# NVIDIA-Genomics-Research/GenomeWorks

Hardware: AMD Instinct MI355X
Metric: cudapoa consensus GCUPS, 1024-window short-read batch (static band 256, 32 reads <= 1024 bp) (higher is better)
Workload: dtype int16; 1 GPU; BASELINE configs[2]: cudapoa single-batch consensus, 1024 windows x 32 reads, backbone 960 bp, <=48 sub/24 ins/24 del, BatchConfig(1024,32,256,static_band), scores 8/-6/-8; windows_per_gpu=1024, cells_per_gpu=10990578176, parallelism=index-split x1

## Files before the change

### genomeworks_amd/csrc/gwhip_poa.hip

```cpp
#include <hip/hip_runtime.h>

#include <cstdio>
#include <cstdlib>
#include <cstring>
#include <string>

#include "poa_device.h"
#include "poa_full_device.h"
#include "poa_graph_device.h"
#include "poa_tb_device.h"

namespace gwhip
{

#ifndef GWHIP_POA_PART
thread_local std::string g_last_error;

static int fail(hipError_t e, const char* what)
{
    g_last_error = std::string(what) + ": " + hipGetErrorString(e);
    return (int)e;
}
static int fail_msg(int code, const std::string& msg)
{
// ... 182 lines not shown
    uint64_t phase_acc[kPhCount] = {0, 0, 0, 0, 0, 0};
    PhaseClock pc{(DBG && a.phase_cycles) ? phase_acc : nullptr, 0};
    wave_sync();
    pc.start();

    for (int32_t s = 1; s < (int32_t)wd.num_seqs; s++)
    {
        const int32_t seq_len = seq_lens[s];
        const int32_t adv     = ((s == 1 ? len0 : seq_lens[s - 1]) + 3) & ~3;
        sequence += adv;
        base_weights += adv;

        if (node_count >= c.max_nodes_per_graph)
        {
            if (lane == 0) { consensus[0] = kKernelError; consensus[1] = kNodeCountExceeded; }
            break;
        }
        pc.tick(kPhOther);
        build_rowinfo<IdT, RowT>(g, node_count, rowinfo, lane, LDS_TABLES ? reinterpret_cast<uint64_t*>(lds_code_tile) : nullptr);
        constexpr bool LDS_READ = LDS_TABLES && BM != GWHIP_FULL_BAND;
        const uint8_t* lds_read = lds_read_buf;
        if constexpr (LDS_READ)
        {
            const int32_t stage_bytes = min(kReadLds, ((max(seq_len, kMaxAdaptiveBand) + 8) + 3) & ~3);
            for (int32_t i = lane * 4; i < stage_bytes; i += kWave * 4)
                *reinterpret_cast<uint32_t*>(lds_read_buf + i) = *reinterpret_cast<const uint32_t*>(sequence + i);
        }
        wave_sync();
        pc.tick(kPhRowInfo);

        int32_t alen = 0;
        constexpr bool kTbPacked = TB && LDS_TABLES && std::is_same<ScoreT, int16_t>::value && std::is_same<TraceT, int16_t>::value;
        bool tb_handled = false;
        if constexpr (kTbPacked)
        {
            constexpr bool kAd = BM == GWHIP_ADAPTIVE_BAND_TRACEBACK;
            const bool adaptive_now = kAd && c.alignment_band_width < kMaxAdaptiveBand;
            auto packed = [&](auto ad_tag, int32_t rerun) -> int32_t {
                return nw_banded_tb_packed<IdT, decltype(ad_tag)::value>(g, rowinfo, node_count, lds_read, seq_len, reinterpret_cast<int16_t*>(scores),
                                                                         a.L.scores_elems, reinterpret_cast<int16_t*>(traceback), a.L.trace_elems,
                                                                         banded_buffer_size, alignment_graph, alignment_read, c.alignment_band_width,
                                                                         c.max_banded_pred_distance, c.gap_score, c.mismatch_score, c.match_score, rerun,
                                                                         cells, smem, kRingBytes, reinterpret_cast<const uint64_t*>(lds_code_tile),
                                                                         debug_flags, tb_handled);
            };
            if (adaptive_now)
                alen = packed(std::integral_constant<bool, kAd>{}, 0);
            else
                alen = packed(std::false_type{}, 0);
        }
        if (tb_handled && !(alen == kShiftLeft || alen == kShiftRight)) {}
        else if (BM == GWHIP_ADAPTIVE_BAND_TRACEBACK && c.alignment_band_width < kMaxAdaptiveBand)
// ... 3 lines not shown
                                                               traceback, a.L.trace_elems, banded_buffer_size, alignment_graph,
                                                               alignment_read, c.alignment_band_width, c.max_banded_pred_distance,
                                                               c.gap_score, c.mismatch_score, c.match_score, alen, cells);
            else
            alen = nw_banded_tb<ScoreT, IdT, RowT, TraceT, true>(g, rowinfo, node_count, sequence, seq_len, scores, a.L.scores_elems,
                                                           traceback, a.L.trace_elems, banded_buffer_size, alignment_graph,
                                                           alignment_read, c.alignment_band_width, c.max_banded_pred_distance,
                                                           c.gap_score, c.mismatch_score, c.match_score, 0, cells);
            if (alen == kShiftLeft || alen == kShiftRight)
                alen = nw_banded_tb<ScoreT, IdT, RowT, TraceT, true>(g, rowinfo, node_count, sequence, seq_len, scores, a.L.scores_elems,
                                                               traceback, a.L.trace_elems, banded_buffer_size, alignment_graph,
                                                               alignment_read, c.alignment_band_width, c.max_banded_pred_distance,
                                                               c.gap_score, c.mismatch_score, c.match_score, alen, cells);
        }
        else if (TB)
        {
            alen = nw_banded_tb<ScoreT, IdT, RowT, TraceT, false>(g, rowinfo, node_count, sequence, seq_len, scores, a.L.scores_elems,
                                                            traceback, a.L.trace_elems, banded_buffer_size, alignment_graph,
                                                            alignment_read, c.alignment_band_width, c.max_banded_pred_distance,
                                                            c.gap_score, c.mismatch_score, c.match_score, 0, cells);
        }
        else if (BM == GWHIP_ADAPTIVE_BAND && c.alignment_band_width < kMaxAdaptiveBand)
        {
            alen = nw_banded<ScoreT, IdT, RowT, true, LDS_READ, PV>(g, rowinfo, node_count, sequence, lds_read, seq_len, scores, ring, ring_bytes,
                                                banded_buffer_size, alignment_graph, alignment_read, c.alignment_band_width,
                                                c.gap_score, c.mismatch_score, c.match_score, 0, cells, pc, debug_flags, codes, lds_code_tile, lds_read_window, lds_bs_ring,
                                                mw_args, mw_shared);
            if (alen == kShiftLeft || alen == kShiftRight)
                alen = nw_banded<ScoreT, IdT, RowT, true, LDS_READ, PV>(g, rowinfo, node_count, sequence, lds_read, seq_len, scores, ring, ring_bytes,
                                                    banded_buffer_size, alignment_graph, alignment_read,
                                                    c.alignment_band_width, c.gap_score, c.mismatch_score, c.match_score,
                                                    alen, cells, pc, debug_flags, codes, lds_code_tile, lds_read_window, lds_bs_ring,
                                                    mw_args, mw_shared);
        }
        else if (BM == GWHIP_STATIC_BAND || BM == GWHIP_ADAPTIVE_BAND)
        {
            alen = nw_banded<ScoreT, IdT, RowT, false, LDS_READ, PV>(g, rowinfo, node_count, sequence, lds_read, seq_len, scores, ring, ring_bytes,
                                                 banded_buffer_size, alignment_graph, alignment_read, c.alignment_band_width,
                                                 c.gap_score, c.mismatch_score, c.match_score, 0, cells, pc, debug_flags, codes, lds_code_tile, lds_read_window, lds_bs_ring);
        }
        else
        {
            bool full_handled = false;
            if constexpr (kFullPacked)
                alen = nw_full_packed<IdT>(g, rowinfo, node_count, sequence, seq_len, reinterpret_cast<int16_t*>(scores), wd.scores_width, full_moves,
                                           smem, kRingBytes, reinterpret_cast<const uint64_t*>(lds_code_tile), alignment_graph, alignment_read,
                                           c.gap_score, c.mismatch_score, c.match_score, cells, debug_flags, full_handled, pc);
            if (!full_handled)
                alen = nw_full<ScoreT, IdT, RowT>(g, rowinfo, node_count, sequence, seq_len, scores, wd.scores_width, ring, kRingBytes,
                                            alignment_graph, alignment_read, c.gap_score, c.mismatch_score, c.match_score, cells);
        }
        alen = (int32_t)(IdT)alen;

        uint8_t err = 0;
        if (alen == kNwLoopFailed) err = kLoopCountExceeded;
        else if (alen == kNwAdaptiveStorageFailed) err = kExceededAdaptiveBandedMatrixSize;
        else if (TB && alen == kNwTracebackBufferFailed) err = kExceededMaximumPredecessorDistance;
        else if (alen == kNwPipelineFailed || alen == kNwScoreWrapped) err = kGenericError;
        if (err)
        {
// ... 6 lines not shown
        int32_t par_rc           = -1;
        if constexpr (!LDS_TABLES && !TB && BM != GWHIP_FULL_BAND)
        {
            int32_t new_count   = 0;
            int32_t* scratch    = reinterpret_cast<int32_t*>(scores);
            const int32_t lpad  = (seq_len + 63) & ~63;
            par_rc = add_alignment_parallel<IdT, MSA, int32_t>(new_count, g, node_count, alen, alignment_graph, alignment_read,
                                                               sequence, base_weights, seq_len, MSA ? g.seq_begin + s : nullptr,
                                                               (uint16_t)s, (uint32_t)c.max_sequences_per_poa,
                                                               c.max_nodes_per_graph, scratch, scratch + lpad,
                                                               reinterpret_cast<uint32_t*>(scratch + 2 * lpad), lane,
                                                               debug_flags, pc.acc ? &pc.acc[kPhOther] : nullptr);
            if (par_rc == 0)
            {
                if (lane == 0) seq_lens[0] = new_count;
                status_and_count = new_count;
            }
            else if (par_rc > 0)
            {
                if (lane == 0) { consensus[0] = kKernelError; consensus[1] = (uint8_t)par_rc; }
                status_and_count = -1;
            }
        }
        if constexpr (LDS_TABLES)
        {
            int32_t new_count = 0;
            par_rc = add_alignment_parallel<IdT, MSA>(new_count, g, node_count, alen, alignment_graph, alignment_read,
                                                      sequence, base_weights, seq_len, MSA ? g.seq_begin + s : nullptr,
                                                      (uint16_t)s, (uint32_t)c.max_sequences_per_poa,
                                                      c.max_nodes_per_graph, reinterpret_cast<int16_t*>(smem),
                                                      reinterpret_cast<int16_t*>(smem) + 2048,
                                                      reinterpret_cast<uint32_t*>(lds_rowinfo_region), lane, debug_flags,
                                                      pc.acc ? &pc.acc[kPhOther] : nullptr);
            if (par_rc == 0)
            {
                if (lane == 0) seq_lens[0] = new_count;
                status_and_count = new_count;
            }
            else if (par_rc > 0)
            {
                if (lane == 0) { consensus[0] = kKernelError; consensus[1] = (uint8_t)par_rc; }
                status_and_count = -1;
            }
        }
        if (lane == 0 && par_rc < 0)
        {
            int32_t new_count = 0;
            uint8_t e = add_alignment_to_graph<IdT, MSA>(new_count, g, node_count, alen, alignment_graph, sequence,
                                                         alignment_read, base_weights, MSA ? g.seq_begin + s : nullptr,
                                                         (uint16_t)s, (uint32_t)c.max_sequences_per_poa,
                                                         (uint32_t)c.max_nodes_per_graph);
            if (e != 0)
            {
                consensus[0]     = kKernelError;
                consensus[1]     = e;
                status_and_count = -1;
            }
            else
            {
                seq_lens[0]      = new_count;
                status_and_count = new_count;
            }
        }
        pc.tick(kPhAddAlignment);
        status_and_count = wave_first(status_and_count);
        constexpr bool kCachedSort = !LDS_TABLES && !TB && BM != GWHIP_FULL_BAND;
        bool sorted_here = false;
        if constexpr (kCachedSort)
        {
            const bool incr_ok = c.max_nodes_per_graph <= 131071 && !(debug_flags & (1 << 17)) &&
                                 (int64_t)a.L.scores_elems * (int64_t)sizeof(ScoreT) >= (int64_t)c.max_nodes_per_graph * 24 + 2048;
// ... 423 lines not shown
    {
        *per_poa    = (int64_t)L.per_window - matrix;
        *per_matrix = matrix;
    }
    *per_poa += (int64_t)cfg->max_consensus_size * 3;
    if (cfg->output_mask & 2) *per_poa += (int64_t)cfg->max_consensus_size * cfg->max_sequences_per_poa;
    *per_poa += (int64_t)cfg->max_sequences_per_poa * cfg->max_sequence_size * 2 + (int64_t)cfg->max_sequences_per_poa * 4 + 32;
}

int32_t gwhip_poa_resident_windows(const gwhip_poa_config* cfg)
{
    if (cfg == nullptr) return 0;
    const bool lds = !cfg->size32 && cfg->max_nodes_per_graph + 2 <= kRowInfoLds && cfg->max_sequence_size + 16 <= kReadLds;
    if (!lds) return 0;
    int cus = 0, dev = 0;
    if (hipGetDevice(&dev) != hipSuccess || hipDeviceGetAttribute(&cus, hipDeviceAttributeMultiprocessorCount, dev) != hipSuccess || cus <= 0)
    {
        (void)hipGetLastError();
        cus = 256;
    }
    return 4 * cus;
}

int gwhip_poa_generate(const gwhip_poa_args* args, gwhip_stream_t stream_)
{
    hipStream_t stream = (hipStream_t)stream_;
    if (!args || !validate(args)) return fail_msg((int)hipErrorInvalidValue, "gwhip_poa_generate: invalid arguments");
    if (args->total_windows == 0) return 0;
    KernelArgs ka = make_kernel_args(args);
    if (!args->workspace || ((uintptr_t)args->workspace & 255) != 0)
        return fail_msg((int)hipErrorInvalidValue, "gwhip_poa_generate: workspace must be 256-byte aligned");
    if (args->workspace_bytes < gwhip_poa_workspace_bytes(&args->cfg, args->total_windows, 0))
        return fail_msg((int)hipErrorInvalidValue, "gwhip_poa_generate: workspace_bytes is smaller than gwhip_poa_workspace_bytes(cfg, total_windows, 0)");
    hipError_t e;
    const bool msa = (args->cfg.output_mask & 2) != 0;
    if (args->cfg.score32)
        e = args->cfg.size32 ? launch_trace_split<int32_t, int32_t>(ka, stream) : launch_trace_split<int32_t, int16_t>(ka, stream);
    else
        e = args->cfg.size32 ? launch_trace_split<int16_t, int32_t>(ka, stream) : launch_trace_split<int16_t, int16_t>(ka, stream);
    if (e != hipSuccess) return fail(e, "poa_window_kernel launch");
    if (args->event_after_graph_build)
    {
        e = hipEventRecord((hipEvent_t)args->event_after_graph_build, stream);
        if (e != hipSuccess) return fail(e, "hipEventRecord");
    }
    dim3 grid(args->total_windows), block(kWave);
// ... 88 lines not shown
```

### genomeworks_amd/cudapoa.py

```python
import ctypes as C

import numpy as np

from . import _native
from .cuda import CudaStream

success = 0
exceeded_maximum_poas = 1
exceeded_maximum_sequence_size = 2
exceeded_maximum_sequences_per_poa = 3
node_count_exceeded_maximum_graph_size = 4
edge_count_exceeded_maximum_graph_size = 5
exceeded_adaptive_banded_matrix_size = 6
exceeded_maximum_predecessor_distance = 7
loop_count_exceeded_upper_bound = 8
output_type_unavailable = 9
zero_weighted_poa_sequence = 10
empty_poa_group = 11
generic_error = 12

_STATUS_NAMES = {
    0: "success", 1: "exceeded_maximum_poas", 2: "exceeded_maximum_sequence_size",
    3: "exceeded_maximum_sequences_per_poa", 4: "node_count_exceeded_maximum_graph_size",
    5: "edge_count_exceeded_maximum_graph_size", 6: "exceeded_adaptive_banded_matrix_size",
# ... 5 lines not shown


def status_to_str(status):
    if status not in _STATUS_NAMES:
        raise RuntimeError("Unknown error status : " + str(status))
    return _STATUS_NAMES[status]


def _bind(L):
    if getattr(L, "_gw_poa_bound", False):
        return L
    vp, i32 = C.c_void_p, C.c_int32
    L.gw_poa_batch_config_full.argtypes = [C.POINTER(_native.PoaBatchConfig)] + [i32] * 8
    L.gw_poa_batch_config_default.argtypes = [C.POINTER(_native.PoaBatchConfig), i32, i32, i32, i32, C.c_float,
                                              C.c_float, i32]
    L.gw_poa_create_batch.restype = vp
    L.gw_poa_create_batch.argtypes = [i32, vp, C.c_int64, C.c_int8, C.POINTER(_native.PoaBatchConfig), C.c_int16,
                                      C.c_int16, C.c_int16]
    L.gw_poa_destroy_batch.argtypes = [vp]
    L.gw_poa_add_poa_group.argtypes = [vp, i32, C.POINTER(C.c_char_p), C.POINTER(vp), C.POINTER(i32), C.POINTER(i32)]
    for name in ("gw_poa_get_total_poas", "gw_poa_generate_poa", "gw_poa_batch_id", "gw_poa_reset", "gw_poa_max_poas",
                 "gw_poa_relaunch"):
        getattr(L, name).argtypes = [vp]
    L.gw_poa_get_consensus.argtypes = [vp, C.POINTER(i32)]
    L.gw_poa_get_consensus_in_place.argtypes = [vp, C.POINTER(i32)]
    L.gw_poa_consensus_str.restype = C.POINTER(C.c_char)
    L.gw_poa_consensus_str.argtypes = [vp, i32, C.POINTER(i32)]
    L.gw_poa_consensus_coverage.restype = C.POINTER(C.c_uint16)
    L.gw_poa_consensus_coverage.argtypes = [vp, i32, C.POINTER(i32)]
    L.gw_poa_output_status.argtypes = [vp, i32]
    L.gw_poa_get_msa.argtypes = [vp, C.POINTER(i32)]
    L.gw_poa_msa_rows.argtypes = [vp, i32]
    L.gw_poa_msa_row.restype = C.POINTER(C.c_char)
    L.gw_poa_msa_row.argtypes = [vp, i32, i32, C.POINTER(i32)]
    L.gw_poa_get_graphs.argtypes = [vp, C.POINTER(i32)]
    L.gw_poa_graph_num_nodes.argtypes = [vp, i32]
    L.gw_poa_graph_num_edges.argtypes = [vp, i32]
    L.gw_poa_graph_copy.argtypes = [vp, i32, vp, vp, vp, vp]
    L.gw_poa_total_cells.argtypes = [vp, C.POINTER(C.c_uint64)]
    L.gw_poa_relaunch_timed.argtypes = [vp, C.POINTER(C.c_float), C.POINTER(C.c_float)]
    L.gw_poa_profile_phases.argtypes = [vp, C.POINTER(C.c_double)]
    L.gw_poa_profile_phases_per_window.argtypes = [vp, C.POINTER(C.c_uint64), C.c_int32]
    L.gw_poa_profile_phases_per_window.restype = C.c_int32
    L._gw_poa_bound = True
    return L

# ... 88 lines not shown
                if w is None:
                    arr[i] = None
                else:
                    a = np.ascontiguousarray(w, dtype=np.int8)
                    keep.append(a)
                    arr[i] = a.ctypes.data
            wptr = arr
        status = self._L.gw_poa_add_poa_group(self._h, n, seqs, wptr, lens, st)
        if status < 0:
            raise RuntimeError(self._L.gw_last_error().decode())
        return (status, list(st) if status not in (exceeded_maximum_poas,) else [])

    @property
    def total_poas(self):
        return self._L.gw_poa_get_total_poas(self._h)

    @property
    def batch_id(self):
        return self._L.gw_poa_batch_id(self._h)

    @property
    def max_poas(self):
        return self._L.gw_poa_max_poas(self._h)

    def generate_poa(self):
        if self._L.gw_poa_generate_poa(self._h) != 0:
            raise RuntimeError(self._L.gw_last_error().decode())

    def relaunch(self):
        if self._L.gw_poa_relaunch(self._h) != 0:
            raise RuntimeError(self._L.gw_last_error().decode())

    def relaunch_timed(self):
        a, b = C.c_float(0), C.c_float(0)
        if self._L.gw_poa_relaunch_timed(self._h, C.byref(a), C.byref(b)) != 0:
            raise RuntimeError(self._L.gw_last_error().decode())
        return a.value, b.value

    def profile_phases(self):
        out = (C.c_double * 6)()
        if self._L.gw_poa_profile_phases(self._h, out) != 0:
            raise RuntimeError(self._L.gw_last_error().decode())
        names = ("row_table", "nw_forward", "sink_traceback", "graph_merge", "topsort", "other")
        return dict(zip(names, [float(x) for x in out]))

    def profile_phases_per_window(self):
# ... 416 lines not shown
```

### genomeworks_amd/host/capi.cpp

```cpp
#include <claraparabricks/genomeworks/cudapoa/batch.hpp>
#include <claraparabricks/genomeworks/cudapoa/cudapoa.hpp>
#include <claraparabricks/genomeworks/cudapoa/utils.hpp>

#include <cstring>
#include <memory>
#include <string>
#include <vector>

#include "../../include/gw_capi.h"
#include "host_common.hpp"
#include "poa_batch_impl.hpp"
#include "aligner_impl.hpp"
#include "aligner_global.hpp"
#include "aligner_semiglobal.hpp"
#include "alignment_impl.hpp"
#include <claraparabricks/genomeworks/cudapoa/multi_device.hpp>
#include <claraparabricks/genomeworks/utils/cudautils.hpp>
#include <stdexcept>
#include <claraparabricks/genomeworks/cudaaligner/aligner.hpp>
#include <claraparabricks/genomeworks/cudaaligner/alignment.hpp>
#include <claraparabricks/genomeworks/cudaaligner/cudaaligner.hpp>
#include <claraparabricks/genomeworks/cudamapper/overlap_alignment.hpp>

namespace gw  = claraparabricks::genomeworks;
// ... 96 lines not shown
    GW_CATCH(nullptr)
}

void gw_poa_destroy_batch(gw_poa_batch* b) { delete b; }

int gw_poa_add_poa_group(gw_poa_batch* b, int32_t n, const char* const* seqs, const int8_t* const* weights,
                         const int32_t* lengths, int32_t* per_seq_status)
{
    GW_TRY
    poa::Group g;
    g.reserve(static_cast<size_t>(n));
    for (int32_t i = 0; i < n; i++) g.push_back(poa::Entry{seqs[i], weights ? weights[i] : nullptr, lengths[i]});
    std::vector<poa::StatusType> st;
    poa::StatusType r = b->batch->add_poa_group(st, g);
    if (per_seq_status)
        for (size_t i = 0; i < st.size() && i < static_cast<size_t>(n); i++) per_seq_status[i] = static_cast<int32_t>(st[i]);
    return static_cast<int>(r);
    GW_CATCH(-1)
}

int32_t gw_poa_get_total_poas(gw_poa_batch* b) { return b->batch->get_total_poas(); }
int32_t gw_poa_batch_id(gw_poa_batch* b) { return b->batch->batch_id(); }
int32_t gw_poa_max_poas(gw_poa_batch* b) { return b->impl ? b->impl->max_poas() : -1; }

int gw_poa_generate_poa(gw_poa_batch* b)
{
    GW_TRY
    b->batch->generate_poa();
    return 0;
    GW_CATCH(-1)
}

int gw_poa_reset(gw_poa_batch* b)
{
    GW_TRY
    b->batch->reset();
    return 0;
    GW_CATCH(-1)
}

int gw_poa_get_consensus(gw_poa_batch* b, int32_t* n_out)
{
    if (n_out) *n_out = 0;
    try
    {
        std::vector<std::string> consensus;
// ... 871 lines not shown
```

### genomeworks_amd/host/cudapoa_batch.cpp

```cpp
#include <claraparabricks/genomeworks/cudapoa/batch.hpp>
#include <claraparabricks/genomeworks/cudapoa/cudapoa.hpp>
#include <claraparabricks/genomeworks/logging/logging.hpp>

#include <algorithm>
#include <thread>
#include <atomic>
#include <climits>
#include <cstdlib>
#include <chrono>
#include <cstring>
#include <iomanip>
#include <stdexcept>
#include <tuple>

#include "../../include/gwhip.h"
#include "alignment_impl.hpp"
#include "host_common.hpp"
#include "owned_hip.hpp"
#include "poa_batch_impl.hpp"

namespace claraparabricks
{
namespace genomeworks
{
// ... 162 lines not shown
    const int64_t avail_mem = std::min(get_size_of_largest_free_memory_block(allocator_), max_mem);
    const int64_t minimum   = per_poa + per_matrix;
    if (avail_mem < minimum) throw requires_at_least(minimum);
    int64_t guess = std::min<int64_t>(avail_mem / (per_poa + per_matrix), INT32_MAX);
    const int64_t per_poa_input = std::max<int64_t>(1, static_cast<int64_t>(max_sequences_per_poa_) *
                                                           cudautils::align<int32_t, 4>(batch_size_.max_sequence_size));
    guess     = std::min<int64_t>(guess, (static_cast<int64_t>(INT32_MAX) - 8192) / per_poa_input);
    max_poas_ = static_cast<int32_t>(std::max<int64_t>(guess, 1));
    while (max_poas_ > 1 && static_cast<int64_t>(plan(max_poas_).block.bytes) > avail_mem) max_poas_--;
    layout_ = plan(max_poas_);
    if (static_cast<int64_t>(layout_.block.bytes) > avail_mem) throw requires_at_least(static_cast<int64_t>(layout_.block.bytes));
    score_buffer_bytes_ = static_cast<size_t>(per_matrix) * static_cast<size_t>(max_poas_);
    workspace_bytes_    = gwhip_poa_workspace_bytes(&cfg_, max_poas_, 0);
    device_block_       = allocator_.allocate(layout_.block.bytes, {stream_});
    d_                  = layout_.in(device_block_);
    input_capacity_     = layout_.sequence_bytes - 4096;
    GW_CU_CHECK_ERR(hipMemsetAsync(d_.sequences, 0, layout_.sequence_bytes, stream_));
    GW_CU_CHECK_ERR(hipMemsetAsync(d_.weights, 0, layout_.sequence_bytes, stream_));
    GW_CU_CHECK_ERR(hipMemsetAsync(d_.work_counters, 0, 256, stream_));

    host_block_ = cudaaligner::pinned_acquire(layout_.workspace.offset, &host_block_capacity_);
    h_          = layout_.in(host_block_);

    live_batches(device_id_).fetch_add(1);
    debug_message(" Initializing batch on device ");
    reset();
}

PoaBatch::~PoaBatch()
{
    debug_message(" Destroyed buffers on device ");
    scoped_device_switch dev(device_id_);
    (void)hipStreamSynchronize(stream_);
    live_batches(device_id_).fetch_sub(1);
    if (host_block_ != nullptr) cudaaligner::pinned_release(host_block_, host_block_capacity_);
    if (device_block_ != nullptr) allocator_.deallocate(device_block_, layout_.block.bytes);
}

void PoaBatch::debug_message(const std::string& message)
{
    std::string msg = std::string(static_cast<size_t>(bid_), '\t') + " " + std::to_string(bid_) + " " + message + " " + std::to_string(device_id_);
    GW_LOG_DEBUG(msg.c_str());
}

PoaBlockLayout PoaBatch::plan(int32_t n_poas) const
{
    const size_t n     = static_cast<size_t>(n_poas);
    const size_t reads = n * static_cast<size_t>(max_sequences_per_poa_);
    const size_t rows  = n * static_cast<size_t>(batch_size_.max_consensus_size);
    PoaBlockLayout l;
    l.sequences      = l.block.take<uint8_t>(reads * static_cast<size_t>(cudautils::align<int32_t, 4>(batch_size_.max_sequence_size)) + 4096);
    l.sequence_bytes = l.block.bytes;
    l.weights        = l.block.take<int8_t>(l.sequence_bytes);
    l.lengths        = l.block.take<int32_t>(reads);
    l.windows        = l.block.take<gwhip_window_details>(n);
    l.consensus      = l.block.take<uint8_t>(rows);
    l.coverage       = l.block.take<uint16_t>(rows);
    l.has_msa        = (output_mask_ & OutputType::msa) != 0;
    l.msa            = l.block.take<uint8_t>(l.has_msa ? rows * static_cast<size_t>(max_sequences_per_poa_) : 0);
    l.cells          = l.block.take<uint64_t>(n);
    l.work_counters  = l.block.take<uint32_t>(64);
    l.workspace      = l.block.take<char>(gwhip_poa_workspace_bytes(&cfg_, n_poas, 0));
    return l;
}

void PoaBatch::reset()
{
    poa_count_              = 0;
    num_nucleotides_copied_ = 0;
    global_sequence_idx_    = 0;
    next_scores_offset_     = 0;
    avail_buf_mem_          = score_buffer_bytes_;
    unit_weights_only_      = true;
}

bool PoaBatch::reserve_buf(int32_t max_seq_length)
{
    const int32_t matrix_height = batch_size_.max_nodes_per_graph;
    const int32_t matrix_width  = (batch_size_.band_mode != BandMode::full_band)
                                      ? batch_size_.matrix_sequence_dimension
                                      : cudautils::align<int32_t, 4>(max_seq_length + 1 + kCellsPerThread);
    size_t required_size        = static_cast<size_t>(matrix_width) * static_cast<size_t>(matrix_height);
    const bool tb               = batch_size_.band_mode == static_band_traceback || batch_size_.band_mode == adaptive_band_traceback;
    required_size *= tb ? (cfg_.trace16 ? 2 : 1) : (cfg_.score32 ? 4 : (batch_size_.band_mode == BandMode::full_band ? 3 : 2));
    if (required_size > avail_buf_mem_)
    {
        if (get_total_poas() == 0)
        {
            std::cout << "Memory available " << std::fixed << std::setprecision(2)
                      << (static_cast<double>(avail_buf_mem_)) / 1024. / 1024. / 1024.;
// ... 63 lines not shown

StatusType PoaBatch::add_poa_group(std::vector<StatusType>& per_seq_status, const Group& poa_group)
{
    if (poa_group.empty())
    {
        per_seq_status.clear();
        return StatusType::empty_poa_group;
    }
    const auto longest = std::max_element(poa_group.begin(), poa_group.end(),
                                          [](const Entry& a, const Entry& b) { return a.length < b.length; });
    {
        int64_t bytes = 0;
        int32_t taken = 0;
        for (const auto& entry : poa_group)
            if (entry.length <= batch_size_.max_sequence_size && taken < max_sequences_per_poa_)
            {
                bytes += cudautils::align<int32_t, 4>(entry.length);
                taken++;
            }
        if (static_cast<int64_t>(num_nucleotides_copied_) + bytes > static_cast<int64_t>(input_capacity_)) return StatusType::exceeded_maximum_poas;
    }
    if (!reserve_buf(longest->length)) return StatusType::exceeded_maximum_poas;
    per_seq_status.clear();
    StatusType status = add_poa();
    if (status != StatusType::success) return status;
    bool poa_empty = true;
    for (const auto& entry : poa_group)
    {
        StatusType entry_status = add_seq_to_poa(entry.seq, entry.weights, entry.length);
        if (entry_status == StatusType::success) poa_empty = false;
        per_seq_status.push_back(entry_status);
    }
    return poa_empty ? StatusType::empty_poa_group : StatusType::success;
}

gwhip_poa_args PoaBatch::kernel_args() const
{
    gwhip_poa_args a{};
    a.cfg              = cfg_;
    a.total_windows    = poa_count_;
    a.sequences        = d_.sequences;
    a.base_weights     = d_.weights;
    a.sequence_lengths = d_.lengths;
    a.window_details   = d_.windows;
    a.consensus        = d_.consensus;
    a.coverage         = d_.coverage;
    a.msa              = d_.msa;
    a.workspace        = layout_.workspace.in(device_block_);
    a.workspace_bytes  = workspace_bytes_;
    a.cells            = d_.cells;
    a.work_counters    = d_.work_counters;
    a.shared_device    = live_batches(device_id_).load(std::memory_order_relaxed) > 1 ? 1 : 0;
    return a;
}

void PoaBatch::upload_inputs()
{
    GW_CU_CHECK_ERR(hipMemcpyAsync(d_.sequences, h_.sequences, static_cast<size_t>(num_nucleotides_copied_), hipMemcpyHostToDevice, stream_));
    if (unit_weights_only_)
        GW_CU_CHECK_ERR(hipMemsetAsync(d_.weights, 1, static_cast<size_t>(num_nucleotides_copied_), stream_));
    else
        GW_CU_CHECK_ERR(hipMemcpyAsync(d_.weights, h_.weights, static_cast<size_t>(num_nucleotides_copied_), hipMemcpyHostToDevice, stream_));
    GW_CU_CHECK_ERR(hipMemsetAsync(d_.sequences + num_nucleotides_copied_, 0, 2048, stream_));
    GW_CU_CHECK_ERR(hipMemcpyAsync(d_.windows, h_.windows, static_cast<size_t>(poa_count_) * sizeof(gwhip_window_details), hipMemcpyHostToDevice, stream_));
    restore_lengths();
}

void PoaBatch::restore_lengths()
{
    GW_CU_CHECK_ERR(hipMemcpyAsync(d_.lengths, h_.lengths, static_cast<size_t>(global_sequence_idx_) * sizeof(int32_t), hipMemcpyHostToDevice, stream_));
}

void PoaBatch::launch(void* event_after_graph_build, uint64_t* phase_cycles)
{
    gwhip_poa_args a          = kernel_args();
    a.event_after_graph_build = event_after_graph_build;
    a.phase_cycles            = phase_cycles;
    const int rc     = gwhip_poa_generate(&a, stream_);
    if (rc != 0)
    {
        char buf[512];
        gwhip_last_error_string(buf, sizeof(buf));
        GW_LOG_ERROR(buf);
        GW_CU_CHECK_ERR(static_cast<hipError_t>(rc));
    }
}

void PoaBatch::generate_poa()
{
    scoped_device_switch dev(device_id_);
    if (poa_count_ == 0)
    {
        debug_message(" No POA was added to compute! ");
        return;
    }
    upload_inputs();
    debug_message(" Launching kernel for " + std::to_string(poa_count_) + " on device ");
    launch();
    debug_message(" Launched kernel on device ");
}

void PoaBatch::relaunch_resident()
{
    scoped_device_switch dev(device_id_);
    if (poa_count_ == 0) return;
    restore_lengths();
    launch();
}

void PoaBatch::relaunch_resident_timed(float* graph_build_ms, float* output_ms)
{
    scoped_device_switch dev(device_id_);
    if (poa_count_ == 0) return;
    gwhost::OwnedEvents events;
    const hipEvent_t e0 = events.create(hipEventDefault), e1 = events.create(hipEventDefault), e2 = events.create(hipEventDefault);
    restore_lengths();
    GW_CU_CHECK_ERR(hipEventRecord(e0, stream_));
    launch(e1);
    GW_CU_CHECK_ERR(hipEventRecord(e2, stream_));
    GW_CU_CHECK_ERR(hipEventSynchronize(e2));
    GW_CU_CHECK_ERR(hipEventElapsedTime(graph_build_ms, e0, e1));
    GW_CU_CHECK_ERR(hipEventElapsedTime(output_ms, e1, e2));
}

void PoaBatch::profile_phases(double out[6])
{
    for (int k = 0; k < 6; k++) out[k] = 0;
    if (poa_count_ == 0) return;
    std::vector<uint64_t> h;
    profile_phases_per_window(h);
    for (size_t i = 0; i < h.size(); i++) out[i % 6] += static_cast<double>(h[i]);
    for (int k = 0; k < 6; k++) out[k] /= poa_count_;
}

void PoaBatch::profile_phases_per_window(std::vector<uint64_t>& ticks)
{
    scoped_device_switch dev(device_id_);
    const size_t n = static_cast<size_t>(poa_count_) * 6;
    ticks.assign(n, 0);
    if (n == 0) return;
    uint64_t* d = nullptr;
    GW_CU_CHECK_ERR(hipMalloc(reinterpret_cast<void**>(&d), n * sizeof(uint64_t)));
    restore_lengths();
    launch(nullptr, d);
    GW_CU_CHECK_ERR(hipMemcpyAsync(ticks.data(), d, n * sizeof(uint64_t), hipMemcpyDeviceToHost, stream_));
    GW_CU_CHECK_ERR(hipStreamSynchronize(stream_));
    GW_CU_CHECK_ERR(hipFree(d));
}

void PoaBatch::log_kernel_error(StatusType error_type)
{
    std::string message, hint;
    decode_error(error_type, message, hint);
    message += " in batch " + std::to_string(bid_) + "\n" + hint;
    GW_LOG_WARN(message.c_str());
}

void PoaBatch::log_failed_windows(const StatusType* status, size_t count)
{
    for (size_t poa = 0; poa < count; poa++)
        if (status[poa] != StatusType::success) log_kernel_error(status[poa]);
}

StatusType PoaBatch::window_status(size_t poa) const
{
// ... 251 lines not shown
```

### genomeworks_amd/host/poa_batch_impl.hpp

```cpp
#pragma once
#include <claraparabricks/genomeworks/cudapoa/batch.hpp>

#include "../../include/gwhip.h"
#include "host_common.hpp"

namespace claraparabricks
{
namespace genomeworks
{
namespace cudapoa
{

gwhip_poa_config make_device_config(const BatchConfig& b, int8_t output_mask, int32_t gap, int32_t mismatch, int32_t match);

void bin_poa_groups(std::vector<BatchConfig>& list_of_batch_sizes, std::vector<std::vector<int32_t>>& list_of_groups_per_batch,
                    const std::vector<int32_t>& capacity, const std::vector<int32_t>& longest, const std::vector<int32_t>& reads,
                    int32_t band_width, BandMode band_mode, float adaptive_storage_factor, float graph_length_factor,
                    int32_t max_pred_distance, const std::vector<int32_t>* bins_capacity);

struct PoaSections
{
    uint8_t* sequences            = nullptr;
    int8_t* weights               = nullptr;
    int32_t* lengths              = nullptr;
// ... 28 lines not shown
    }
};

class PoaBatch : public Batch
{
public:
    PoaBatch(int32_t device_id, cudaStream_t stream, DefaultDeviceAllocator allocator, int64_t max_mem, int8_t output_mask,
             const BatchConfig& batch_size, int32_t gap_score = -8, int32_t mismatch_score = -6, int32_t match_score = 8);
    ~PoaBatch() override;

    StatusType add_poa_group(std::vector<StatusType>& per_seq_status, const Group& poa_group) override;
    int32_t get_total_poas() const override { return poa_count_; }
    void generate_poa() override;
    StatusType get_consensus(std::vector<std::string>& consensus, std::vector<std::vector<uint16_t>>& coverage,
                             std::vector<StatusType>& output_status) override;
    StatusType get_msa(std::vector<std::vector<std::string>>& msa, std::vector<StatusType>& output_status) override;
    void get_graphs(std::vector<DirectedGraph>& graphs, std::vector<StatusType>& output_status) override;
    int32_t batch_id() const override { return bid_; }
    void reset() override;

    StatusType get_consensus_in_place(std::vector<std::string>& consensus, std::vector<std::vector<uint16_t>>& coverage,
                                      std::vector<StatusType>& output_status);
    int32_t max_poas() const { return max_poas_; }
    uint64_t total_cells();
    void relaunch_resident();
    void relaunch_resident_timed(float* graph_build_ms, float* output_ms);
    void profile_phases(double out[6]);
    void profile_phases_per_window(std::vector<uint64_t>& ticks);
    const gwhip_poa_config& device_config() const { return cfg_; }
    cudaStream_t stream() const { return stream_; }

private:
    void debug_message(const std::string& message);
    bool reserve_buf(int32_t max_seq_length);
    StatusType add_poa();
    StatusType add_seq_to_poa(const char* seq, const int8_t* weights, int32_t seq_len);
    void upload_inputs();
    void restore_lengths();
    void launch(void* event_after_graph_build = nullptr, uint64_t* phase_cycles = nullptr);
    gwhip_poa_args kernel_args() const;
    StatusType window_status(size_t poa) const;
    void log_kernel_error(StatusType error_type);
    void log_failed_windows(const StatusType* status, size_t count);
    void fetch_consensus(std::string* consensus, std::vector<uint16_t>* coverage, StatusType* output_status, bool presize);
    PoaBlockLayout plan(int32_t n_poas) const;

    int32_t max_sequences_per_poa_ = 0;
    int32_t device_id_             = 0;
    cudaStream_t stream_           = nullptr;
    int8_t output_mask_            = 0;
    BatchConfig batch_size_;
    DefaultDeviceAllocator allocator_;
    gwhip_poa_config cfg_{};
    int32_t bid_      = 0;
    int32_t max_poas_ = 0;

    int32_t poa_count_              = 0;
    int32_t num_nucleotides_copied_ = 0;
    bool unit_weights_only_         = true;
    int32_t global_sequence_idx_    = 0;
    size_t avail_buf_mem_           = 0;
    size_t next_scores_offset_      = 0;
    size_t score_buffer_bytes_      = 0;

    PoaBlockLayout layout_;
    size_t workspace_bytes_ = 0;
    size_t input_capacity_  = 0;
    char* device_block_     = nullptr;
    PoaSections d_;
    char* host_block_           = nullptr;
    size_t host_block_capacity_ = 0;
    PoaSections h_;
};

}
}
}
```

### include/gw_capi.h

```cpp
#ifndef GW_CAPI_H
#define GW_CAPI_H

#include <stddef.h>
#include <stdint.h>

#ifdef __cplusplus
extern "C" {
#endif

typedef struct gw_poa_batch gw_poa_batch;
typedef struct gw_aligner gw_aligner;

const char* gw_last_error(void);

int gw_device_count(int* count);
int gw_set_device(int device);
int gw_get_device(int* device);
int gw_mem_info(size_t* free_bytes, size_t* total_bytes);
int gw_stream_create(void** stream);
int gw_stream_sync(void* stream);
int gw_stream_destroy(void* stream);

int64_t gw_generate_window(uint32_t seed, int32_t backbone_len, int32_t n_reads, int32_t max_mut, int32_t max_ins,
                           int32_t max_del, char* out, int64_t out_cap, int32_t* lens);
// ... 14 lines not shown
    int32_t band_mode;
    int32_t max_banded_pred_distance;
} gw_poa_batch_config;

int gw_poa_batch_config_default(gw_poa_batch_config* out, int32_t max_seq_sz, int32_t max_seq_per_poa,
                                int32_t band_width, int32_t band_mode, float adaptive_storage_factor,
                                float graph_length_factor, int32_t max_pred_dist);
int gw_poa_batch_config_full(gw_poa_batch_config* out, int32_t max_seq_sz, int32_t max_consensus_sz,
                             int32_t max_nodes_per_poa, int32_t band_width, int32_t max_seq_per_poa,
                             int32_t matrix_seq_dim, int32_t band_mode, int32_t max_pred_distance);

gw_poa_batch* gw_poa_create_batch(int32_t device_id, void* stream, int64_t max_mem, int8_t output_mask,
                                  const gw_poa_batch_config* cfg, int16_t gap_score, int16_t mismatch_score,
                                  int16_t match_score);
void gw_poa_destroy_batch(gw_poa_batch* b);

int gw_poa_add_poa_group(gw_poa_batch* b, int32_t n, const char* const* seqs, const int8_t* const* weights,
                         const int32_t* lengths, int32_t* per_seq_status);
int32_t gw_poa_get_total_poas(gw_poa_batch* b);
int gw_poa_generate_poa(gw_poa_batch* b);
int32_t gw_poa_batch_id(gw_poa_batch* b);
int gw_poa_reset(gw_poa_batch* b);
int32_t gw_poa_max_poas(gw_poa_batch* b);

int gw_poa_get_consensus(gw_poa_batch* b, int32_t* n_out);
int gw_poa_get_consensus_in_place(gw_poa_batch* b, int32_t* n_out);
const char* gw_poa_consensus_str(gw_poa_batch* b, int32_t poa, int32_t* length);
const uint16_t* gw_poa_consensus_coverage(gw_poa_batch* b, int32_t poa, int32_t* length);
int32_t gw_poa_output_status(gw_poa_batch* b, int32_t poa);

int gw_poa_get_msa(gw_poa_batch* b, int32_t* n_out);
int32_t gw_poa_msa_rows(gw_poa_batch* b, int32_t poa);
const char* gw_poa_msa_row(gw_poa_batch* b, int32_t poa, int32_t row, int32_t* length);

int gw_poa_get_graphs(gw_poa_batch* b, int32_t* n_out);
int32_t gw_poa_graph_num_nodes(gw_poa_batch* b, int32_t poa);
int32_t gw_poa_graph_num_edges(gw_poa_batch* b, int32_t poa);
int gw_poa_graph_copy(gw_poa_batch* b, int32_t poa, char* node_labels, int32_t* edge_src, int32_t* edge_dst,
                      int32_t* edge_weight);

int gw_poa_total_cells(gw_poa_batch* b, uint64_t* cells);
int gw_poa_relaunch(gw_poa_batch* b);
int gw_poa_relaunch_timed(gw_poa_batch* b, float* graph_build_ms, float* output_ms);
int gw_poa_profile_phases(gw_poa_batch* b, double* out6);
int gw_poa_profile_phases_per_window(gw_poa_batch* b, uint64_t* out, int32_t capacity_windows);

// ... 97 lines not shown
```

### include/gwhip.h

```cpp
#ifndef GWHIP_H
#define GWHIP_H

#include <stddef.h>
#include <stdint.h>

#ifdef __cplusplus
extern "C" {
#endif

typedef void* gwhip_stream_t;

#define GWHIP_MAX_NODE_EDGES 50
#define GWHIP_MAX_NODE_ALIGNMENTS 50

enum gwhip_band_mode
{
    GWHIP_FULL_BAND = 0,
    GWHIP_STATIC_BAND,
    GWHIP_ADAPTIVE_BAND,
    GWHIP_STATIC_BAND_TRACEBACK,
    GWHIP_ADAPTIVE_BAND_TRACEBACK
};

typedef struct gwhip_window_details
// ... 28 lines not shown
    gwhip_poa_config cfg;
    int32_t total_windows;
    const uint8_t* sequences;
    const int8_t* base_weights;
    int32_t* sequence_lengths;
    const gwhip_window_details* window_details;
    uint8_t* consensus;
    uint16_t* coverage;
    uint8_t* msa;
    void* workspace;
    size_t workspace_bytes;
    uint64_t* cells;
    void* event_after_graph_build;
    uint64_t* phase_cycles;
    uint32_t* work_counters;
    int32_t shared_device;
} gwhip_poa_args;

size_t gwhip_poa_workspace_bytes(const gwhip_poa_config* cfg, int32_t windows, uint64_t sum_scores_width);

void gwhip_poa_bytes_per_window(const gwhip_poa_config* cfg, int64_t* per_poa, int64_t* per_matrix);

int32_t gwhip_poa_resident_windows(const gwhip_poa_config* cfg);

int gwhip_poa_generate(const gwhip_poa_args* args, gwhip_stream_t stream);

int gwhip_poa_export_graphs(const gwhip_poa_args* args, uint8_t* nodes, int32_t* incoming_edges,
                            uint16_t* incoming_edge_weights, uint16_t* incoming_edge_count, int32_t* outgoing_edges,
                            uint16_t* outgoing_edge_count, gwhip_stream_t stream);
int gwhip_poa_export_graphs_range(const gwhip_poa_args* args, int32_t first_window, int32_t n_windows, uint8_t* nodes,
                                  int32_t* incoming_edges, uint16_t* incoming_edge_weights, uint16_t* incoming_edge_count,
                                  int32_t* outgoing_edges, uint16_t* outgoing_edge_count, gwhip_stream_t stream);

typedef struct gwhip_poa_test_graph
{
    const uint8_t* nodes;
    const int32_t* graph;
    const int32_t* node_id_to_pos;
    int32_t graph_count;
    const uint16_t* incoming_edge_count;
    const int32_t* incoming_edges;
    const uint16_t* outgoing_edge_count;
    const int32_t* outgoing_edges;
} gwhip_poa_test_graph;

size_t gwhip_poa_test_nw_scratch_bytes(const gwhip_poa_config* cfg);
// ... 116 lines not shown
```

Baseline: 433.4 GCUPS.

## Read POA sequences directly from mapped pinned host memory, skipping the H2D copy

In the LDS-staged banded path the kernel now reads sequences straight from pinned host memory through a device-mapped pointer, so the host-to-device memcpy of sequences is skipped. The banded and merge steps take their read from the LDS copy, so host memory is only touched while staging. Staging now uses 16-byte vector loads instead of 4-byte ones. Events and lazy re-upload keep host buffer reuse and the resident relaunch paths correct, at the cost of PCIe-latency reads inside the kernel.

After: 443.6 GCUPS (median of 6 runs). 2.4% higher.

```diff
diff --git a/genomeworks_amd/csrc/gwhip_poa.hip b/genomeworks_amd/csrc/gwhip_poa.hip
--- a/genomeworks_amd/csrc/gwhip_poa.hip
+++ b/genomeworks_amd/csrc/gwhip_poa.hip
@@ -228,12 +228,16 @@
         const uint8_t* lds_read = lds_read_buf;
         if constexpr (LDS_READ)
         {
+            typedef uint32_t StageVec __attribute__((ext_vector_type(4)));
+            typedef StageVec StageVecA4 __attribute__((aligned(4)));
+            static_assert(kReadLds % 16 == 0 && (kRingBytes + kRowInfoBytes) % 16 == 0, "16-byte fetches fill the LDS copy of the read");
             const int32_t stage_bytes = min(kReadLds, ((max(seq_len, kMaxAdaptiveBand) + 8) + 3) & ~3);
-            for (int32_t i = lane * 4; i < stage_bytes; i += kWave * 4)
-                *reinterpret_cast<uint32_t*>(lds_read_buf + i) = *reinterpret_cast<const uint32_t*>(sequence + i);
+            for (int32_t i = lane * 16; i < stage_bytes; i += kWave * 16)
+                *reinterpret_cast<StageVec*>(lds_read_buf + i) = *reinterpret_cast<const StageVecA4*>(sequence + i);
         }
         wave_sync();
         pc.tick(kPhRowInfo);
+        const uint8_t* banded_read = LDS_READ ? lds_read : sequence;
 
         int32_t alen = 0;
         constexpr bool kTbPacked = TB && LDS_TABLES && std::is_same<ScoreT, int16_t>::value && std::is_same<TraceT, int16_t>::value;
@@ -283,12 +287,12 @@
         }
         else if (BM == GWHIP_ADAPTIVE_BAND && c.alignment_band_width < kMaxAdaptiveBand)
         {
-            alen = nw_banded<ScoreT, IdT, RowT, true, LDS_READ, PV>(g, rowinfo, node_count, sequence, lds_read, seq_len, scores, ring, ring_bytes,
+            alen = nw_banded<ScoreT, IdT, RowT, true, LDS_READ, PV>(g, rowinfo, node_count, banded_read, lds_read, seq_len, scores, ring, ring_bytes,
                                                 banded_buffer_size, alignment_graph, alignment_read, c.alignment_band_width,
                                                 c.gap_score, c.mismatch_score, c.match_score, 0, cells, pc, debug_flags, codes, lds_code_tile, lds_read_window, lds_bs_ring,
                                                 mw_args, mw_shared);
             if (alen == kShiftLeft || alen == kShiftRight)
-                alen = nw_banded<ScoreT, IdT, RowT, true, LDS_READ, PV>(g, rowinfo, node_count, sequence, lds_read, seq_len, scores, ring, ring_bytes,
+                alen = nw_banded<ScoreT, IdT, RowT, true, LDS_READ, PV>(g, rowinfo, node_count, banded_read, lds_read, seq_len, scores, ring, ring_bytes,
                                                     banded_buffer_size, alignment_graph, alignment_read,
                                                     c.alignment_band_width, c.gap_score, c.mismatch_score, c.match_score,
                                                     alen, cells, pc, debug_flags, codes, lds_code_tile, lds_read_window, lds_bs_ring,
@@ -296,7 +300,7 @@
         }
         else if (BM == GWHIP_STATIC_BAND || BM == GWHIP_ADAPTIVE_BAND)
         {
-            alen = nw_banded<ScoreT, IdT, RowT, false, LDS_READ, PV>(g, rowinfo, node_count, sequence, lds_read, seq_len, scores, ring, ring_bytes,
+            alen = nw_banded<ScoreT, IdT, RowT, false, LDS_READ, PV>(g, rowinfo, node_count, banded_read, lds_read, seq_len, scores, ring, ring_bytes,
                                                  banded_buffer_size, alignment_graph, alignment_read, c.alignment_band_width,
                                                  c.gap_score, c.mismatch_score, c.match_score, 0, cells, pc, debug_flags, codes, lds_code_tile, lds_read_window, lds_bs_ring);
         }
@@ -349,11 +353,12 @@
                 status_and_count = -1;
             }
         }
+        const uint8_t* merge_read = (LDS_READ && !TB) ? lds_read : sequence;
         if constexpr (LDS_TABLES)
         {
             int32_t new_count = 0;
             par_rc = add_alignment_parallel<IdT, MSA>(new_count, g, node_count, alen, alignment_graph, alignment_read,
-                                                      sequence, base_weights, seq_len, MSA ? g.seq_begin + s : nullptr,
+                                                      merge_read, base_weights, seq_len, MSA ? g.seq_begin + s : nullptr,
                                                       (uint16_t)s, (uint32_t)c.max_sequences_per_poa,
                                                       c.max_nodes_per_graph, reinterpret_cast<int16_t*>(smem),
                                                       reinterpret_cast<int16_t*>(smem) + 2048,
@@ -373,7 +378,7 @@
         if (lane == 0 && par_rc < 0)
         {
             int32_t new_count = 0;
-            uint8_t e = add_alignment_to_graph<IdT, MSA>(new_count, g, node_count, alen, alignment_graph, sequence,
+            uint8_t e = add_alignment_to_graph<IdT, MSA>(new_count, g, node_count, alen, alignment_graph, merge_read,
                                                          alignment_read, base_weights, MSA ? g.seq_begin + s : nullptr,
                                                          (uint16_t)s, (uint32_t)c.max_sequences_per_poa,
                                                          (uint32_t)c.max_nodes_per_graph);
@@ -843,6 +848,13 @@
     return 4 * cus;
 }
 
+int32_t gwhip_poa_reads_host_sequences(const gwhip_poa_config* cfg)
+{
+    if (cfg == nullptr) return 0;
+    const bool lds = !cfg->size32 && cfg->max_nodes_per_graph + 2 <= kRowInfoLds && cfg->max_sequence_size + 16 <= kReadLds;
+    return lds && (cfg->band_mode == GWHIP_STATIC_BAND || cfg->band_mode == GWHIP_ADAPTIVE_BAND) ? 1 : 0;
+}
+
 int gwhip_poa_generate(const gwhip_poa_args* args, gwhip_stream_t stream_)
 {
     hipStream_t stream = (hipStream_t)stream_;
diff --git a/genomeworks_amd/cudapoa.py b/genomeworks_amd/cudapoa.py
--- a/genomeworks_amd/cudapoa.py
+++ b/genomeworks_amd/cudapoa.py
@@ -51,6 +51,9 @@
     for name in ("gw_poa_get_total_poas", "gw_poa_generate_poa", "gw_poa_batch_id", "gw_poa_reset", "gw_poa_max_poas",
                  "gw_poa_relaunch"):
         getattr(L, name).argtypes = [vp]
+    if hasattr(L, "gw_poa_last_generate_read_host"):
+        L.gw_poa_last_generate_read_host.argtypes = [vp]
+        L.gw_poa_last_generate_read_host.restype = i32
     L.gw_poa_get_consensus.argtypes = [vp, C.POINTER(i32)]
     L.gw_poa_get_consensus_in_place.argtypes = [vp, C.POINTER(i32)]
     L.gw_poa_consensus_str.restype = C.POINTER(C.c_char)
@@ -185,6 +188,10 @@
     @property
     def max_poas(self):
         return self._L.gw_poa_max_poas(self._h)
+
+    @property
+    def last_generate_read_host(self):
+        return self._L.gw_poa_last_generate_read_host(self._h) == 1
 
     def generate_poa(self):
         if self._L.gw_poa_generate_poa(self._h) != 0:
diff --git a/genomeworks_amd/host/capi.cpp b/genomeworks_amd/host/capi.cpp
--- a/genomeworks_amd/host/capi.cpp
+++ b/genomeworks_amd/host/capi.cpp
@@ -142,6 +142,7 @@
 int32_t gw_poa_get_total_poas(gw_poa_batch* b) { return b->batch->get_total_poas(); }
 int32_t gw_poa_batch_id(gw_poa_batch* b) { return b->batch->batch_id(); }
 int32_t gw_poa_max_poas(gw_poa_batch* b) { return b->impl ? b->impl->max_poas() : -1; }
+int32_t gw_poa_last_generate_read_host(gw_poa_batch* b) { return b->impl ? (b->impl->last_generate_read_host() ? 1 : 0) : -1; }
 
 int gw_poa_generate_poa(gw_poa_batch* b)
 {
diff --git a/genomeworks_amd/host/cudapoa_batch.cpp b/genomeworks_amd/host/cudapoa_batch.cpp
--- a/genomeworks_amd/host/cudapoa_batch.cpp
+++ b/genomeworks_amd/host/cudapoa_batch.cpp
@@ -208,6 +208,15 @@
     host_block_ = cudaaligner::pinned_acquire(layout_.workspace.offset, &host_block_capacity_);
     h_          = layout_.in(host_block_);
 
+    if (gwhip_poa_reads_host_sequences(&cfg_) != 0)
+    {
+        void* mapped = nullptr;
+        if (hipHostGetDevicePointer(&mapped, h_.sequences, 0) == hipSuccess)
+            host_sequences_dev_ = static_cast<const uint8_t*>(mapped);
+        else
+            (void)hipGetLastError();
+    }
+
     live_batches(device_id_).fetch_add(1);
     debug_message(" Initializing batch on device ");
     reset();
@@ -218,6 +227,9 @@
     debug_message(" Destroyed buffers on device ");
     scoped_device_switch dev(device_id_);
     (void)hipStreamSynchronize(stream_);
+    if (host_reads_pending_) (void)hipEventSynchronize(static_cast<hipEvent_t>(host_reads_done_));
+    host_reads_pending_ = false;
+    if (host_reads_done_ != nullptr) (void)hipEventDestroy(static_cast<hipEvent_t>(host_reads_done_));
     live_batches(device_id_).fetch_sub(1);
     if (host_block_ != nullptr) cudaaligner::pinned_release(host_block_, host_block_capacity_);
     if (device_block_ != nullptr) allocator_.deallocate(device_block_, layout_.block.bytes);
@@ -250,8 +262,17 @@
     return l;
 }
 
+void PoaBatch::wait_for_host_reads()
+{
+    if (!host_reads_pending_) return;
+    GW_CU_CHECK_ERR(hipEventSynchronize(static_cast<hipEvent_t>(host_reads_done_)));
+    host_reads_pending_ = false;
+}
+
 void PoaBatch::reset()
 {
+    wait_for_host_reads();
+    device_sequences_current_ = false;
     poa_count_              = 0;
     num_nucleotides_copied_ = 0;
     global_sequence_idx_    = 0;
@@ -361,6 +382,8 @@
     }
     if (!reserve_buf(longest->length)) return StatusType::exceeded_maximum_poas;
     per_seq_status.clear();
+    wait_for_host_reads();
+    device_sequences_current_ = false;
     StatusType status = add_poa();
     if (status != StatusType::success) return status;
     bool poa_empty = true;
@@ -393,14 +416,40 @@
     return a;
 }
 
-void PoaBatch::upload_inputs()
+bool PoaBatch::use_host_input() const
+{
+    if (host_sequences_dev_ == nullptr) return false;
+    const char* e = std::getenv("GW_POA_HOST_INPUT");
+    return !(e != nullptr && e[0] == '0');
+}
+
+void PoaBatch::upload_sequences()
 {
     GW_CU_CHECK_ERR(hipMemcpyAsync(d_.sequences, h_.sequences, static_cast<size_t>(num_nucleotides_copied_), hipMemcpyHostToDevice, stream_));
+    GW_CU_CHECK_ERR(hipMemsetAsync(d_.sequences + num_nucleotides_copied_, 0, 2048, stream_));
+    device_sequences_current_ = true;
+}
+
+void PoaBatch::ensure_resident_sequences()
+{
+    if (!device_sequences_current_) upload_sequences();
+}
+
+void PoaBatch::upload_inputs(bool host_input)
+{
+    if (!host_input)
+        GW_CU_CHECK_ERR(hipMemcpyAsync(d_.sequences, h_.sequences, static_cast<size_t>(num_nucleotides_copied_), hipMemcpyHostToDevice, stream_));
     if (unit_weights_only_)
         GW_CU_CHECK_ERR(hipMemsetAsync(d_.weights, 1, static_cast<size_t>(num_nucleotides_copied_), stream_));
     else
         GW_CU_CHECK_ERR(hipMemcpyAsync(d_.weights, h_.weights, static_cast<size_t>(num_nucleotides_copied_), hipMemcpyHostToDevice, stream_));
-    GW_CU_CHECK_ERR(hipMemsetAsync(d_.sequences + num_nucleotides_copied_, 0, 2048, stream_));
+    if (!host_input)
+    {
+        GW_CU_CHECK_ERR(hipMemsetAsync(d_.sequences + num_nucleotides_copied_, 0, 2048, stream_));
+        device_sequences_current_ = true;
+    }
+    else
+        std::memset(h_.sequences + num_nucleotides_copied_, 0, 2048);
     GW_CU_CHECK_ERR(hipMemcpyAsync(d_.windows, h_.windows, static_cast<size_t>(poa_count_) * sizeof(gwhip_window_details), hipMemcpyHostToDevice, stream_));
     restore_lengths();
 }
@@ -410,9 +459,10 @@
     GW_CU_CHECK_ERR(hipMemcpyAsync(d_.lengths, h_.lengths, static_cast<size_t>(global_sequence_idx_) * sizeof(int32_t), hipMemcpyHostToDevice, stream_));
 }
 
-void PoaBatch::launch(void* event_after_graph_build, uint64_t* phase_cycles)
+void PoaBatch::launch(void* event_after_graph_build, uint64_t* phase_cycles, const uint8_t* sequences)
 {
     gwhip_poa_args a          = kernel_args();
+    if (sequences != nullptr) a.sequences = sequences;
     a.event_after_graph_build = event_after_graph_build;
     a.phase_cycles            = phase_cycles;
     const int rc     = gwhip_poa_generate(&a, stream_);
@@ -433,9 +483,27 @@
         debug_message(" No POA was added to compute! ");
         return;
     }
-    upload_inputs();
+    const bool host_input    = use_host_input();
+    last_generate_read_host_ = host_input;
+    if (host_input)
+    {
+        wait_for_host_reads();
+        if (host_reads_done_ == nullptr)
+        {
+            hipEvent_t e = nullptr;
+            GW_CU_CHECK_ERR(hipEventCreateWithFlags(&e, hipEventDisableTiming));
+            host_reads_done_ = e;
+        }
+    }
+    upload_inputs(host_input);
     debug_message(" Launching kernel for " + std::to_string(poa_count_) + " on device ");
-    launch();
+    if (host_input)
+    {
+        host_reads_pending_ = true;
+        launch(host_reads_done_, nullptr, host_sequences_dev_);
+    }
+    else
+        launch();
     debug_message(" Launched kernel on device ");
 }
 
@@ -443,6 +511,7 @@
 {
     scoped_device_switch dev(device_id_);
     if (poa_count_ == 0) return;
+    ensure_resident_sequences();
     restore_lengths();
     launch();
 }
@@ -453,6 +522,7 @@
     if (poa_count_ == 0) return;
     gwhost::OwnedEvents events;
     const hipEvent_t e0 = events.create(hipEventDefault), e1 = events.create(hipEventDefault), e2 = events.create(hipEventDefault);
+    ensure_resident_sequences();
     restore_lengths();
     GW_CU_CHECK_ERR(hipEventRecord(e0, stream_));
     launch(e1);
@@ -480,6 +550,7 @@
     if (n == 0) return;
     uint64_t* d = nullptr;
     GW_CU_CHECK_ERR(hipMalloc(reinterpret_cast<void**>(&d), n * sizeof(uint64_t)));
+    ensure_resident_sequences();
     restore_lengths();
     launch(nullptr, d);
     GW_CU_CHECK_ERR(hipMemcpyAsync(ticks.data(), d, n * sizeof(uint64_t), hipMemcpyDeviceToHost, stream_));
diff --git a/genomeworks_amd/host/poa_batch_impl.hpp b/genomeworks_amd/host/poa_batch_impl.hpp
--- a/genomeworks_amd/host/poa_batch_impl.hpp
+++ b/genomeworks_amd/host/poa_batch_impl.hpp
@@ -74,6 +74,7 @@
     StatusType get_consensus_in_place(std::vector<std::string>& consensus, std::vector<std::vector<uint16_t>>& coverage,
                                       std::vector<StatusType>& output_status);
     int32_t max_poas() const { return max_poas_; }
+    bool last_generate_read_host() const { return last_generate_read_host_; }
     uint64_t total_cells();
     void relaunch_resident();
     void relaunch_resident_timed(float* graph_build_ms, float* output_ms);
@@ -87,9 +88,13 @@
     bool reserve_buf(int32_t max_seq_length);
     StatusType add_poa();
     StatusType add_seq_to_poa(const char* seq, const int8_t* weights, int32_t seq_len);
-    void upload_inputs();
+    void upload_inputs(bool host_input);
+    void upload_sequences();
+    void ensure_resident_sequences();
     void restore_lengths();
-    void launch(void* event_after_graph_build = nullptr, uint64_t* phase_cycles = nullptr);
+    void launch(void* event_after_graph_build = nullptr, uint64_t* phase_cycles = nullptr, const uint8_t* sequences = nullptr);
+    bool use_host_input() const;
+    void wait_for_host_reads();
     gwhip_poa_args kernel_args() const;
     StatusType window_status(size_t poa) const;
     void log_kernel_error(StatusType error_type);
@@ -123,6 +128,12 @@
     char* host_block_           = nullptr;
     size_t host_block_capacity_ = 0;
     PoaSections h_;
+
+    const uint8_t* host_sequences_dev_ = nullptr;
+    bool device_sequences_current_ = false;
+    void* host_reads_done_         = nullptr;
+    bool host_reads_pending_       = false;
+    bool last_generate_read_host_  = false;
 };
 
 }
diff --git a/include/gw_capi.h b/include/gw_capi.h
--- a/include/gw_capi.h
+++ b/include/gw_capi.h
@@ -60,6 +60,7 @@
 int32_t gw_poa_batch_id(gw_poa_batch* b);
 int gw_poa_reset(gw_poa_batch* b);
 int32_t gw_poa_max_poas(gw_poa_batch* b);
+int32_t gw_poa_last_generate_read_host(gw_poa_batch* b);
 
 int gw_poa_get_consensus(gw_poa_batch* b, int32_t* n_out);
 int gw_poa_get_consensus_in_place(gw_poa_batch* b, int32_t* n_out);
diff --git a/include/gwhip.h b/include/gwhip.h
--- a/include/gwhip.h
+++ b/include/gwhip.h
@@ -74,6 +74,8 @@
 void gwhip_poa_bytes_per_window(const gwhip_poa_config* cfg, int64_t* per_poa, int64_t* per_matrix);
 
 int32_t gwhip_poa_resident_windows(const gwhip_poa_config* cfg);
+
+int32_t gwhip_poa_reads_host_sequences(const gwhip_poa_config* cfg);
 
 int gwhip_poa_generate(const gwhip_poa_args* args, gwhip_stream_t stream);
 
```
